# NVlabs/ODISE

Measured on NVIDIA H100. Metric: images/sec @1024x1024 panoptic inference (ODISE hot path), higher is better.
Workload: dtype f16q8

## Files before the change

odise_b200/csrc/gemm_tc.cu:

```cuda
#include "ptx.cuh"
#include "wgmma.cuh"
#include "odise_b200.h"
#include "launch_count.h"
#include <cudaTypedefs.h>
#include <mutex>
#include <map>
#include <cstring>
#include <vector>
#include <cstdlib>
#include <cstdio>

namespace ob {

struct GemmParams {
  int M, N, K, batch;
  int a_batched, b_batched;
  int conv, C, H, W, bw, bh, bb;
  int nseg;
  int cstride, cpad;
  int tiles_m, tiles_n, splits, kblocks;
  float alpha;
  const float* bias;
  const float* bias_m;
  const float* rowbias;
// ... 129 lines not shown
    float* d = p.D + (long long)z * p.d_bs + (long long)m * p.ldd + n;
    if (vec) {
      *reinterpret_cast<float4*>(d) = make_float4(acc[0], acc[1], acc[2], acc[3]);
    } else {
#pragma unroll
      for (int j = 0; j < 4; ++j) if (j < valid) d[j] = acc[j];
    }
  }
  if (p.Dh) {
    __nv_bfloat16* dh = p.Dh + (long long)z * p.h_bs + (long long)m * p.ldh + n;
    __nv_bfloat16* dl = p.Dl ? p.Dl + (long long)z * p.h_bs + (long long)m * p.ldh + n : nullptr;
    if (p.h16) {
      __align__(8) __nv_bfloat16 h[4];
      __align__(8) __nv_bfloat16 l[4];
#pragma unroll
      for (int t = 0; t < 4; ++t)
        split_f16(acc[t], *reinterpret_cast<uint16_t*>(&h[t]), *reinterpret_cast<uint16_t*>(&l[t]));
      if (vec) {
        *reinterpret_cast<uint2*>(dh) = *reinterpret_cast<const uint2*>(h);
        if (dl) *reinterpret_cast<uint2*>(dl) = *reinterpret_cast<const uint2*>(l);
      } else {
#pragma unroll
        for (int j = 0; j < 4; ++j) if (j < valid) { dh[j] = h[j]; if (dl) dl[j] = l[j]; }
      }
    } else if (vec) {
      store_planes<4>(dh, dl, acc);
    } else {
#pragma unroll
      for (int j = 0; j < 4; ++j) if (j < valid) store_planes<1>(dh + j, dl ? dl + j : nullptr, acc + j);
    }
  }
}

template <int BN, int NMMA>
struct GemmCfg {
  static constexpr int BM = 128, BK = 64;
  static constexpr int A_BYTES = BM * BK * 2;
  static constexpr int B_BYTES = BN * BK * 2;
  static constexpr int PLANES = (NMMA == 1) ? 1 : 2;
  static constexpr int STAGE_BYTES = PLANES * (A_BYTES + B_BYTES);
  static constexpr int THREADS = 384;
  static constexpr int EPI_BYTES = 8 * 32 * 16 * 4;
  static constexpr int STAGES_RAW = (232448 - EPI_BYTES - 256 - 1024) / STAGE_BYTES;
  static constexpr int STAGES = STAGES_RAW > 8 ? 8 : STAGES_RAW;
  static constexpr int SMEM_BYTES = STAGES * STAGE_BYTES + EPI_BYTES + 256 + 1024;
  static_assert(STAGES >= 2, "GEMM tile does not fit shared memory");
};

template <int BN, int NMMA, int EPI>
__global__ void __launch_bounds__(GemmCfg<BN, NMMA>::THREADS, 1)
gemm_tc_kernel(const __grid_constant__ CUtensorMap tmAh, const __grid_constant__ CUtensorMap tmAl,
               const __grid_constant__ CUtensorMap tmBh, const __grid_constant__ CUtensorMap tmBl, const GemmParams p) {
  using Cfg = GemmCfg<BN, NMMA>;
  extern __shared__ uint8_t smem_raw[];
  uint8_t* smem = reinterpret_cast<uint8_t*>((reinterpret_cast<uintptr_t>(smem_raw) + 1023) & ~uintptr_t(1023));
  float* epi_smem = reinterpret_cast<float*>(smem + Cfg::STAGES * Cfg::STAGE_BYTES);
  uint64_t* bars = reinterpret_cast<uint64_t*>(smem + Cfg::STAGES * Cfg::STAGE_BYTES + Cfg::EPI_BYTES);
  uint64_t* full = bars;
  uint64_t* empty = bars + Cfg::STAGES;

  const int warp = threadIdx.x >> 5;
  const int lane = threadIdx.x & 31;

  if (warp == 8 && lane == 0) {
    tma_prefetch_desc(&tmAh);
    tma_prefetch_desc(&tmBh);
    if (NMMA != 1) {
      tma_prefetch_desc(&tmAl);
      tma_prefetch_desc(&tmBl);
    }
    for (int s = 0; s < Cfg::STAGES; ++s) {
      mbar_init(&full[s], 1);
      mbar_init(&empty[s], 8);
    }
    fence_barrier_init();
  }
  __syncthreads();

  const int tiles_per_z = p.tiles_m * p.tiles_n * p.splits;
  const int total_tiles = tiles_per_z * p.batch;
  const int kb_per_split = (p.kblocks + p.splits - 1) / p.splits;

  if (warp >= 8) {
    setmaxnreg_dec<40>();
    if (warp == 8 && lane == 0) {
      int stage = 0;
      uint32_t phase = 0;
      const int cpk = p.conv ? (p.C / 64) : 1;
      for (int tile = blockIdx.x; tile < total_tiles; tile += gridDim.x) {
        const int z = tile / tiles_per_z;
        int r = tile - z * tiles_per_z;
        const int sp = r / (p.tiles_m * p.tiles_n);
        r -= sp * (p.tiles_m * p.tiles_n);
        const int mt = r / p.tiles_n, nt = r % p.tiles_n;
        const int m0 = mt * 128, n0 = nt * BN;
        const int kb0 = sp * kb_per_split;
        const int kb1 = min(p.kblocks, kb0 + kb_per_split);
        int b0 = 0, h0 = 0, w0 = 0;
        if (p.conv) {
          const int hw = p.H * p.W;
          b0 = m0 / hw;
          const int rem = m0 - b0 * hw;
          h0 = rem / p.W;
          w0 = rem - h0 * p.W;
        }
        for (int kb = kb0; kb < kb1; ++kb) {
          mbar_wait(&empty[stage], phase ^ 1);
          uint8_t* st = smem + stage * Cfg::STAGE_BYTES;
          mbar_arrive_expect_tx(&full[stage], Cfg::STAGE_BYTES);
          if (p.conv) {
            const int tap = kb / cpk, cc = kb - tap * cpk;
            const int kh = tap / 3, kw = tap - kh * 3;
            if (p.nseg == 1) {
              const int cx = w0 * p.cstride + kw - p.cpad, cy = h0 * p.cstride + kh - p.cpad;
              tma_load_4d(st, &tmAh, &full[stage], cc * 64, cx, cy, b0);
              if (NMMA != 1) tma_load_4d(st + Cfg::A_BYTES, &tmAl, &full[stage], cc * 64, cx, cy, b0);
            } else {
              const int hw = p.H * p.W;
              for (int sg = 0; sg < p.nseg; ++sg) {
                const int m = m0 + sg * p.bw;
                const int bi = m / hw, rem = m - bi * hw;
                const int hi_ = rem / p.W, wi = rem - hi_ * p.W;
                const int cx = wi * p.cstride + kw - p.cpad, cy = hi_ * p.cstride + kh - p.cpad;
                uint8_t* sa = st + sg * p.bw * 128;
                tma_load_4d(sa, &tmAh, &full[stage], cc * 64, cx, cy, bi);
                if (NMMA != 1) tma_load_4d(sa + Cfg::A_BYTES, &tmAl, &full[stage], cc * 64, cx, cy, bi);
              }
            }
          } else {
            const int za = p.a_batched ? z : 0;
            tma_load_3d(st, &tmAh, &full[stage], kb * 64, m0, za);
            if (NMMA != 1) tma_load_3d(st + Cfg::A_BYTES, &tmAl, &full[stage], kb * 64, m0, za);
          }
          const int zb = p.b_batched ? z : 0;
          uint8_t* sb = st + Cfg::PLANES * Cfg::A_BYTES;
          tma_load_3d(sb, &tmBh, &full[stage], kb * 64, n0, zb);
          if (NMMA != 1) tma_load_3d(sb + Cfg::B_BYTES, &tmBl, &full[stage], kb * 64, n0, zb);
          if (++stage == Cfg::STAGES) { stage = 0; phase ^= 1; }
        }
      }
    }
    return;
  }

  setmaxnreg_inc<232>();
  const int wg = warp >> 2, wi = warp & 3;
  int stage = 0;
  uint32_t phase = 0;
  float acc[BN / 2];
  float acc2[BN / 2];
  float* stg_wg = epi_smem + wg * (4 * 512);
  float* stg = stg_wg + wi * 512;
  const int cq = lane & 3, rsub = lane >> 2;
  for (int tile = blockIdx.x; tile < total_tiles; tile += gridDim.x) {
    const int z = tile / tiles_per_z;
    int r = tile - z * tiles_per_z;
    const int sp = r / (p.tiles_m * p.tiles_n);
    r -= sp * (p.tiles_m * p.tiles_n);
    const int mt = r / p.tiles_n, nt = r % p.tiles_n;
    const int n0 = nt * BN;
    const int kb0 = sp * kb_per_split;
    const int kb1 = min(p.kblocks, kb0 + kb_per_split);

    if (kb0 >= kb1) {
#pragma unroll
      for (int i = 0; i < BN / 2; ++i) acc[i] = 0.f;
      if constexpr (NMMA == 2) {
#pragma unroll
        for (int i = 0; i < BN / 2; ++i) acc2[i] = 0.f;
      }
    }
    int prev = -1;
    for (int kb = kb0; kb < kb1; ++kb) {
      mbar_wait(&full[stage], phase);
      const uint32_t sa = smem_u32(smem + stage * Cfg::STAGE_BYTES) + wg * (64 * 128);
      const uint32_t sb = smem_u32(smem + stage * Cfg::STAGE_BYTES + Cfg::PLANES * Cfg::A_BYTES);
      reg_fence(acc);
      if constexpr (NMMA == 2) reg_fence(acc2);
      wgmma_fence();
#pragma unroll
      for (int k = 0; k < 4; ++k) {
        const uint64_t a_hi = wgmma_desc_sw128(sa + k * 32);
        const uint64_t b_hi = wgmma_desc_sw128(sb + k * 32);
        const int accum = (kb > kb0 || k > 0) ? 1 : 0;
        if constexpr (NMMA == 2) wgmma_f16(acc, a_hi, b_hi, accum);
        else wgmma_bf16(acc, a_hi, b_hi, accum);
        if constexpr (NMMA == 3) {
          wgmma_bf16(acc, a_hi, wgmma_desc_sw128(sb + Cfg::B_BYTES + k * 32), 1);
          wgmma_bf16(acc, wgmma_desc_sw128(sa + Cfg::A_BYTES + k * 32), b_hi, 1);
        }
      }
      if constexpr (NMMA == 2) {
        const uint32_t a2 = sa + Cfg::A_BYTES, b2 = sb + Cfg::B_BYTES;
#pragma unroll
        for (int k = 0; k < 2; ++k) {
          wgmma_e5m2(acc2, wgmma_desc_sw128(a2 + k * 32), wgmma_desc_sw128(b2 + 64 + k * 32), (kb > kb0 || k > 0) ? 1 : 0);
          wgmma_e5m2(acc2, wgmma_desc_sw128(a2 + 64 + k * 32), wgmma_desc_sw128(b2 + k * 32), 1);
        }
      }
      wgmma_commit();
      wgmma_wait<1>();
      if (prev >= 0 && lane == 0) mbar_arrive(&empty[prev]);
      prev = stage;
      if (++stage == Cfg::STAGES) { stage = 0; phase ^= 1; }
    }
    wgmma_wait<0>();
    reg_fence(acc);
    if (prev >= 0 && lane == 0) mbar_arrive(&empty[prev]);
    if constexpr (NMMA == 2) {
      reg_fence(acc2);
#pragma unroll
      for (int i = 0; i < BN / 2; ++i) acc[i] += acc2[i];
    }

    const int m_base = mt * 128 + wg * 64 + (wi & 1) * 32;
    const bool interior = p.vec_ok && p.splits == 1 && (mt * 128 + 128 <= p.M) && (n0 + BN <= p.N);
    constexpr bool EXTRA = EPI == 1, GEGLU = EPI == 2;
    const bool has_bias = p.bias != nullptr, has_res = EXTRA && p.res != nullptr;
    const bool to_f32 = p.D != nullptr, to_hi = p.Dh != nullptr, to_lo = p.Dl != nullptr;
    const int act = p.act;
    const float alpha = p.alpha;
    const bool has_gn = !GEGLU && p.gnp != nullptr;
    const long long gn_seg = ((long long)z * p.M + m_base) >> 5;
#pragma unroll 1
    for (int ch = 0; ch < BN / 32; ++ch) {
      named_bar_sync(1 + wg, 128);
#pragma unroll
      for (int j = 0; j < BN / 8; ++j) {
        if ((j >> 2) != ch) continue;
#pragma unroll
        for (int h = 0; h < 2; ++h) {
          const int rw = wi * 16 + rsub + 8 * h, cc = 8 * (j & 3) + 2 * cq;
          const int rr = rw & 31, c16 = cc & 15;
          float* dst = stg_wg + ((rw >> 5) | ((cc >> 4) << 1)) * 512 + rr * 16 + (((c16 >> 2) ^ ((rr >> 1) & 3)) << 2) + (c16 & 3);
          *reinterpret_cast<float2*>(dst) = make_float2(acc[4 * j + 2 * h], acc[4 * j + 2 * h + 1]);
        }
      }
      named_bar_sync(1 + wg, 128);
      const int c0 = ch * 32 + (wi >> 1) * 16;
      if (interior) {
        GnAcc gacc;
        float4 b4 = make_float4(0.f, 0.f, 0.f, 0.f);
        if (has_bias) b4 = __ldg(reinterpret_cast<const float4*>(p.bias + n0 + c0 + cq * 4));
        float4 q[4];
#pragma unroll
        for (int it = 0; it < 4; ++it) {
          const int rr = it * 8 + rsub;
          q[it] = *reinterpret_cast<const float4*>(stg + rr * 16 + ((cq ^ ((rr >> 1) & 3)) << 2));
        }
        const int nn = n0 + c0 + cq * 4;
        float4 r4[4];
        if (has_res) {
#pragma unroll
          for (int it = 0; it < 4; ++it)
            r4[it] = *reinterpret_cast<const float4*>(p.res + (long long)z * p.res_bs + (long long)(m_base + it * 8 + rsub) * p.ldres + nn);
        }
#pragma unroll
        for (int it = 0; it < 4; ++it) {
          const long long m = m_base + it * 8 + rsub;
          float e[4] = {q[it].x, q[it].y, q[it].z, q[it].w};
          const float bb[4] = {b4.x, b4.y, b4.z, b4.w};
          const float bm = (EXTRA && p.bias_m) ? __ldg(p.bias_m + m) : 0.f;
#pragma unroll
          for (int j = 0; j < 4; ++j) e[j] = fmaf(e[j], alpha, EXTRA ? bb[j] + bm : bb[j]);
          if (EXTRA && p.rowbias) {
            const float4 rb = __ldg(reinterpret_cast<const float4*>(
                p.rowbias + (((long long)z * p.M + m) / p.rows_per_group) * p.rowbias_ld + nn));
            e[0] += rb.x; e[1] += rb.y; e[2] += rb.z; e[3] += rb.w;
          }
          if (GEGLU) {
            const bool odd = cq & 1;
            const float r0 = __shfl_xor_sync(0xffffffffu, odd ? e[0] : e[2], 1);
            const float r1 = __shfl_xor_sync(0xffffffffu, odd ? e[1] : e[3], 1);
            const float a0 = odd ? r0 : e[0], a1 = odd ? r1 : e[1];
            const float g0 = odd ? e[2] : r0, g1 = odd ? e[3] : r1;
            const float gv[2] = {a0 * gelu_erf_fast(g0), a1 * gelu_erf_fast(g1)};
            const long long og = (long long)z * p.h_bs + m * p.ldh + ((n0 + c0) >> 1) + (cq >> 1) * 4 + (odd ? 2 : 0);
            store_planes<2>(p.Dh + og, to_lo ? p.Dl + og : nullptr, gv);
            continue;
          }
          if (act != ODISE_ACT_NONE) {
#pragma unroll
            for (int j = 0; j < 4; ++j) e[j] = apply_act(e[j], act);
          }
          if (has_res) { e[0] += r4[it].x; e[1] += r4[it].y; e[2] += r4[it].z; e[3] += r4[it].w; }
          if (has_gn) gn_acc_rows(gacc, e, it == 0, lane);
          if (to_f32) *reinterpret_cast<float4*>(p.D + (long long)z * p.d_bs + m * p.ldd + nn) = make_float4(e[0], e[1], e[2], e[3]);
          const long long oh = (long long)z * p.h_bs + m * p.ldh + nn;
          if (to_hi && p.h16) {
            const __half2 h01 = __floats2half2_rn(e[0], e[1]), h23 = __floats2half2_rn(e[2], e[3]);
            uint2 hv;
            hv.x = *reinterpret_cast<const uint32_t*>(&h01);
            hv.y = *reinterpret_cast<const uint32_t*>(&h23);
            *reinterpret_cast<uint2*>(p.Dh + oh) = hv;
            if (to_lo) {
              const float2 f01 = __half22float2(h01), f23 = __half22float2(h23);
              const __half2 l01 = __floats2half2_rn(e[0] - f01.x, e[1] - f01.y);
              const __half2 l23 = __floats2half2_rn(e[2] - f23.x, e[3] - f23.y);
              uint2 lv;
              lv.x = *reinterpret_cast<const uint32_t*>(&l01);
              lv.y = *reinterpret_cast<const uint32_t*>(&l23);
              *reinterpret_cast<uint2*>(p.Dl + oh) = lv;
            }
          } else if (to_hi) {
            store_planes<4>(p.Dh + oh, to_lo ? p.Dl + oh : nullptr, e);
          }
        }
        if (has_gn) gn_acc_store(gacc, p, gn_seg, n0 + c0 + cq * 4, 4, lane);
      } else if (n0 + c0 < p.N) {
        const bool gn_here = p.gnp != nullptr && !p.geglu && p.splits == 1 && m_base < p.M;
        GnAcc gacc;
#pragma unroll 1
        for (int it = 0; it < 4; ++it) {
          const int rr = it * 8 + rsub;
          const float4 q4 = *reinterpret_cast<const float4*>(stg + rr * 16 + ((cq ^ ((rr >> 1) & 3)) << 2));
          const int m = m_base + rr, n = n0 + c0 + cq * 4;
          if (p.geglu) {
            float e[4] = {q4.x, q4.y, q4.z, q4.w};
#pragma unroll
            for (int j = 0; j < 4; ++j) e[j] = fmaf(e[j], p.alpha, p.bias ? __ldg(p.bias + n + j) : 0.f);
            float gt[4];
#pragma unroll
            for (int j = 0; j < 4; ++j) gt[j] = __shfl_xor_sync(0xffffffffu, e[j], 1);
            if ((cq & 1) == 0 && m < p.M) {
              float gv[4];
#pragma unroll
              for (int t = 0; t < 4; ++t) gv[t] = e[t] * gelu_erf_fast(gt[t]);
              const long long og = (long long)z * p.h_bs + (long long)m * p.ldh + ((n0 + c0) >> 1) + (cq >> 1) * 4;
              store_planes<4>(p.Dh + og, p.Dl ? p.Dl + og : nullptr, gv);
            }
            continue;
          }
          float fin[4] = {0.f, 0.f, 0.f, 0.f};
          if (m < p.M && n < p.N) {
            const int valid = min(4, p.N - n);
            if (p.splits > 1) {
              float* dst = p.partial + ((long long)(sp * p.batch + z) * p.M + m) * p.N + n;
              const float e[4] = {q4.x, q4.y, q4.z, q4.w};
#pragma unroll
              for (int j = 0; j < 4; ++j) if (j < valid) dst[j] = e[j];
            } else {
              epilogue_quad(p, z, m, n, valid, q4, fin);
            }
          }
          if (gn_here) gn_acc_rows(gacc, fin, it == 0, lane);
        }
        if (gn_here) {
          const int n = n0 + c0 + cq * 4;
          gn_acc_store(gacc, p, ((long long)z * p.M + m_base) >> 5, n, n < p.N ? min(4, p.N - n) : 0, lane);
        }
      }
    }
  }
}

__global__ void gemm_splitk_reduce_kernel(const GemmParams p) {
  const int quads = (p.N + 3) / 4;
  const long long total = (long long)p.batch * p.M * quads;
  for (long long i = blockIdx.x * (long long)blockDim.x + threadIdx.x; i < total;
       i += (long long)gridDim.x * blockDim.x) {
    const int qd = (int)(i % quads);
    const long long zm = i / quads;
    const int m = (int)(zm % p.M);
    const int z = (int)(zm / p.M);
    const int n = qd * 4;
    const int valid = min(4, p.N - n);
    float acc[4] = {0.f, 0.f, 0.f, 0.f};
    for (int sp = 0; sp < p.splits; ++sp) {
      const float* src = p.partial + ((long long)(sp * p.batch + z) * p.M + m) * p.N + n;
#pragma unroll
      for (int j = 0; j < 4; ++j) if (j < valid) acc[j] += src[j];
    }
    epilogue_quad(p, z, m, n, valid, make_float4(acc[0], acc[1], acc[2], acc[3]));
  }
}

static PFN_cuTensorMapEncodeTiled_v12000 get_encode() {
  static PFN_cuTensorMapEncodeTiled_v12000 fn = nullptr;
  static std::once_flag once;
  std::call_once(once, [] {
    void* f = nullptr;
    cudaDriverEntryPointQueryResult q;
    if (cudaGetDriverEntryPoint("cuTensorMapEncodeTiled", &f, cudaEnableDefault, &q) == cudaSuccess &&
        q == cudaDriverEntryPointSuccess)
      fn = reinterpret_cast<PFN_cuTensorMapEncodeTiled_v12000>(f);
  });
  return fn;
}

static int encode_map(CUtensorMap* tm, const void* base, int rank, const cuuint64_t* dims,
                      const cuuint64_t* strides_bytes, const cuuint32_t* box, int spatial_stride = 1) {
  auto enc = get_encode();
  if (!enc) return ODISE_ERR_DRIVER;
  cuuint32_t estr[5] = {1, (cuuint32_t)spatial_stride, (cuuint32_t)spatial_stride, 1, 1};
  CUresult r = enc(tm, CU_TENSOR_MAP_DATA_TYPE_BFLOAT16, rank, const_cast<void*>(base), dims, strides_bytes, box,
                   estr, CU_TENSOR_MAP_INTERLEAVE_NONE, CU_TENSOR_MAP_SWIZZLE_128B,
                   CU_TENSOR_MAP_L2_PROMOTION_L2_256B, CU_TENSOR_MAP_FLOAT_OOB_FILL_NONE);
  return r == CUDA_SUCCESS ? ODISE_OK : ODISE_ERR_TENSORMAP;
}

struct ProfRec { cudaEvent_t a, b; double flops; int M, N, K, batch, conv, bn, nmma, splits; };
static std::vector<ProfRec> g_prof;
static bool g_prof_on = false;

int num_sms() {
  static int n = 0;
  if (!n) {
    int dev = 0;
    cudaGetDevice(&dev);
    cudaDeviceGetAttribute(&n, cudaDevAttrMultiProcessorCount, dev);
    if (n <= 0) n = 132;
  }
  return n;
}

template <int BN, int NMMA, int EPI>
static int launch_cfg(const CUtensorMap& ah, const CUtensorMap& al, const CUtensorMap& bh, const CUtensorMap& bl,
                      const GemmParams& p, cudaStream_t stream) {
  using Cfg = GemmCfg<BN, NMMA>;
  static bool attr_set = false;
  if (!attr_set) {
    cudaError_t e = cudaFuncSetAttribute(gemm_tc_kernel<BN, NMMA, EPI>, cudaFuncAttributeMaxDynamicSharedMemorySize,
                                         Cfg::SMEM_BYTES);
    if (e != cudaSuccess) return (int)e;
    attr_set = true;
  }
  const int total = p.tiles_m * p.tiles_n * p.splits * p.batch;
  const int grid = total < num_sms() ? total : num_sms();
  gemm_tc_kernel<BN, NMMA, EPI><<<grid, Cfg::THREADS, Cfg::SMEM_BYTES, stream>>>(ah, al, bh, bl, p);
  return (int)cudaGetLastError();
}

static int pick_tile(int M, int N, int K, int batch, int forced, bool conv, int nmma) {
  const int cands[4] = {256, 160, 128, 64};
  const double eff[4] = {0.833, 0.933, 1.0, 1.333};
  const double epi_k = 480.0;
  const long long tm = (M + 127) / 128;
  double best = 1e30;
  int c = 128;
  for (int i = 0; i < 4; ++i) {
    const int bn = cands[i];
    if (forced && bn != forced) continue;
    if (nmma == 2 && bn > 128) continue;
    const long long tn = (N + bn - 1) / bn;
    const long long units = tm * tn * batch;
    const long long waves = (units + num_sms() - 1) / num_sms();
    double cost;
    if (conv) {
      cost = (double)waves * bn * eff[i] + 0.02 * bn;
    } else {
      const double mma = (double)bn * K * eff[i], epi = (double)bn * epi_k;
      cost = (double)waves * ((mma > epi ? mma : epi) + 20000.0);
    }
    if (cost < best) { best = cost; c = bn; }
  }
  return c;
}

}

using namespace ob;

// ... 91 lines not shown
    if (d->lda % 8 || d->a_batch_stride % 8) return ODISE_ERR_ALIGN;
    const long long bs = d->a_batch_stride ? d->a_batch_stride : (long long)d->M * d->lda;
    cuuint64_t dims[3] = {(cuuint64_t)d->K, (cuuint64_t)d->M, (cuuint64_t)(d->a_batch_stride ? d->batch : 1)};
    cuuint64_t str[2] = {(cuuint64_t)d->lda * 2, (cuuint64_t)bs * 2};
    cuuint32_t box[3] = {64, 128, 1};
    rc = encode_map(&ah, d->a_hi, 3, dims, str, box);
    if (rc) return rc;
    if (d->nmma == 2) {
      dims[0] = (cuuint64_t)((d->K + 63) / 64 * 64);
      if ((long long)dims[0] > d->lda) return ODISE_ERR_ALIGN;
    }
    rc = encode_map(&al, d->nmma != 1 ? d->a_lo : d->a_hi, 3, dims, str, box);
    if (rc) return rc;
  }
  p.tiles_m = (d->M + 127) / 128;
  if (d->ldb % 8 || d->b_batch_stride % 8) return ODISE_ERR_ALIGN;
  if (d->nmma == 2 && (long long)((d->K + 63) / 64 * 64) > d->ldb) return ODISE_ERR_ALIGN;
  if (d->geglu) {
    if (!d->out_hi || d->out_f32 || d->residual || d->rowbias || d->bias_m || d->split_k > 1 || d->N % 16 ||
        !p.vec_ok || d->act != ODISE_ACT_NONE)
      return ODISE_ERR_UNSUPPORTED;
  }
  p.kblocks = (d->K + 63) / 64;
  p.splits = d->split_k > 1 ? d->split_k : 1;
  if (p.splits > p.kblocks) p.splits = p.kblocks;
  if (p.splits > 1) {
    if (!d->workspace ||
        d->workspace_bytes < (long long)p.splits * d->batch * d->M * d->N * (long long)sizeof(float))
      return ODISE_ERR_WORKSPACE;
    p.partial = reinterpret_cast<float*>(d->workspace);
  }
  const int epi = d->geglu ? 2 : ((d->residual || d->rowbias || d->bias_m) ? 1 : 0);

  auto launch_with = [&](int bn) -> int {
    p.tiles_n = (d->N + bn - 1) / bn;
    const long long bs = d->b_batch_stride ? d->b_batch_stride : (long long)d->N * d->ldb;
    cuuint64_t dims[3] = {(cuuint64_t)d->K, (cuuint64_t)d->N, (cuuint64_t)(d->b_batch_stride ? d->batch : 1)};
    cuuint64_t str[2] = {(cuuint64_t)d->ldb * 2, (cuuint64_t)bs * 2};
    cuuint32_t box[3] = {64, (cuuint32_t)bn, 1};
    int r = encode_map(&bh, d->b_hi, 3, dims, str, box);
    if (r) return r;
    if (d->nmma == 2) dims[0] = (cuuint64_t)((d->K + 63) / 64 * 64);
    r = encode_map(&bl, d->nmma != 1 ? d->b_lo : d->b_hi, 3, dims, str, box);
    if (r) return r;
#define ODISE_LAUNCH(BN_, NM_)                                                   \
  r = epi == 2   ? launch_cfg<BN_, NM_, 2>(ah, al, bh, bl, p, stream)            \
      : epi == 1 ? launch_cfg<BN_, NM_, 1>(ah, al, bh, bl, p, stream)            \
                 : launch_cfg<BN_, NM_, 0>(ah, al, bh, bl, p, stream)
    if (d->nmma == 3) {
      switch (bn) {
        case 64: ODISE_LAUNCH(64, 3); break;
        case 128: ODISE_LAUNCH(128, 3); break;
        case 160: ODISE_LAUNCH(160, 3); break;
        default: ODISE_LAUNCH(256, 3); break;
      }
    } else if (d->nmma == 2) {
      if (bn == 64) ODISE_LAUNCH(64, 2);
      else ODISE_LAUNCH(128, 2);
    } else {
      switch (bn) {
        case 64: ODISE_LAUNCH(64, 1); break;
        case 128: ODISE_LAUNCH(128, 1); break;
        case 160: ODISE_LAUNCH(160, 1); break;
        default: ODISE_LAUNCH(256, 1); break;
      }
    }
#undef ODISE_LAUNCH
    if (r) return r;
    if (p.splits > 1) {
      const long long total = (long long)p.batch * p.M * ((p.N + 3) / 4);
      int blocks = (int)((total + 127) / 128);
      if (blocks > num_sms() * 8) blocks = num_sms() * 8;
      gemm_splitk_reduce_kernel<<<blocks, 128, 0, stream>>>(p);
      r = (int)cudaGetLastError();
    }
    return r;
  };

  int BN;
  {
    static const bool tune = !(getenv("ODISE_GEMM_AUTOTUNE") && atoi(getenv("ODISE_GEMM_AUTOTUNE")) == 0);
    const int fbn = (d->force_bn == 64 || d->force_bn == 128 || d->force_bn == 160 || d->force_bn == 256) ? d->force_bn : 0;
    BN = pick_tile(d->M, d->N, d->K, d->batch, fbn, d->conv3x3 != 0, d->nmma);
    struct Key {
      int v[13];
      bool operator<(const Key& o) const { return memcmp(v, o.v, sizeof(v)) < 0; }
    };
    static std::map<Key, int> cache;
    static std::mutex mu;
    const Key key{{d->M, d->N, d->K, d->batch, d->conv3x3 ? 1 + d->conv_mode : 0, d->conv_W, d->nmma, epi, p.splits,
                  (d->out_f32 ? 1 : 0) | (d->out_hi ? 2 : 0) | (d->out_planes_fp16 << 2), p.gnp ? 1 : 0, d->act, p.vec_ok}};
    cudaStreamCaptureStatus cap = cudaStreamCaptureStatusNone;
    cudaStreamIsCapturing(stream, &cap);
    std::lock_guard<std::mutex> lk(mu);
    auto it = cache.find(key);
    if (it != cache.end()) {
      BN = it->second;
    } else if (tune && !fbn && !g_prof_on && cap == cudaStreamCaptureStatusNone &&
               !(d->residual && (const void*)d->residual == (const void*)d->out_f32)) {
      const int cands[4] = {256, 160, 128, 64};
      cudaEvent_t e0, e1;
      cudaEventCreate(&e0);
      cudaEventCreate(&e1);
      float best = 1e30f;
      int bc = BN;
      for (int i = 0; i < 4; ++i) {
        const int c = cands[i];
        if (c == 64 && d->N > 96 && (long long)p.tiles_m * ((d->N + 127) / 128) * d->batch >= 2 * num_sms()) continue;
        if (c > 128 && (d->N <= 64 || d->nmma == 2)) continue;
        if (launch_with(c)) { (void)cudaGetLastError(); continue; }
        cudaEventRecord(e0, stream);
        int r2 = launch_with(c);
        if (!r2) r2 = launch_with(c);
        cudaEventRecord(e1, stream);
        if (r2 || cudaEventSynchronize(e1) != cudaSuccess) { (void)cudaGetLastError(); continue; }
        float ms = 0.f;
        cudaEventElapsedTime(&ms, e0, e1);
        if (ms < best) { best = ms; bc = c; }
      }
      cudaEventDestroy(e0);
      cudaEventDestroy(e1);
      cache[key] = bc;
      BN = bc;
      if (getenv("ODISE_VERBOSE"))
        fprintf(stderr, "odise_b200: gemm %d x %d x %d (batch %d, conv %d, nmma %d, epi %d): BN %d, %.1f us\n", d->M, d->N,
                d->K, d->batch, d->conv3x3, d->nmma, epi, BN, best * 500.f);
    }
  }

  ProfRec rec{};
  if (g_prof_on) {
    cudaEventCreate(&rec.a);
    cudaEventCreate(&rec.b);
    rec.flops = 2.0 * d->M * d->N * (double)d->K * d->batch;
    rec.M = d->M; rec.N = d->N; rec.K = d->K; rec.batch = d->batch; rec.conv = d->conv3x3; rec.bn = BN;
    rec.nmma = d->nmma; rec.splits = p.splits;
    cudaEventRecord(rec.a, stream);
  }
  rc = launch_with(BN);
  if (rc) return rc;
  count_launch(p.splits > 1 ? 2 : 1);
  if (g_prof_on) {
    cudaEventRecord(rec.b, stream);
    g_prof.push_back(rec);
  }
  return rc;
}

extern "C" int odise_gemm_tile_policy(int M, int N, int K, int batch, int conv3x3, int nmma, int* bn, int* pair) {
  if (M <= 0 || N <= 0 || K <= 0 || batch <= 0 || !bn || !pair || nmma < 1 || nmma > 3) return ODISE_ERR_ARG;
  *bn = pick_tile(M, N, K, batch, 0, conv3x3 != 0, nmma);
  *pair = 0;
  return ODISE_OK;
}

extern "C" int odise_profile_begin(void) {
  for (auto& r : g_prof) { cudaEventDestroy(r.a); cudaEventDestroy(r.b); }
  g_prof.clear();
  g_prof_on = true;
  return ODISE_OK;
}

extern "C" int odise_profile_end(long long* launches, double* total_ms, double* total_flops) {
  g_prof_on = false;
  cudaError_t e = cudaDeviceSynchronize();
  if (e != cudaSuccess) return (int)e;
  double ms = 0, fl = 0;
  FILE* fcsv = nullptr;
  if (const char* path = getenv("ODISE_PROFILE_CSV")) fcsv = fopen(path, "a");
  if (fcsv) fprintf(fcsv, "M,N,K,batch,conv,bn,nmma,splits,ms,tflops\n");
  for (auto& r : g_prof) {
    float t = 0;
// ... 16 lines not shown
```

Before: 12.41.

## Add warp-specialized epilogue variant that hands accumulators to dedicated epilogue warps

Adds a HAND variant of the TMA/WGMMA GEMM. Consumer warpgroups dump accumulator chunks into shared-memory slots guarded by mbarriers. Three otherwise idle producer-group warps then run the bias/activation/residual/GN epilogue, with residual loads prefetched before waiting, so the epilogue overlaps the next tile's MMAs. The autotuner now times both variants per BN, and the extra staging slots can reduce pipeline stages, and register rebalancing via setmaxnreg is skipped in this mode.

```diff
diff --git a/odise_b200/csrc/gemm_tc.cu b/odise_b200/csrc/gemm_tc.cu
--- a/odise_b200/csrc/gemm_tc.cu
+++ b/odise_b200/csrc/gemm_tc.cu
@@ -185,7 +185,7 @@
   }
 }
 
-template <int BN, int NMMA>
+template <int BN, int NMMA, bool HAND>
 struct GemmCfg {
   static constexpr int BM = 128, BK = 64;
   static constexpr int A_BYTES = BM * BK * 2;
@@ -193,24 +193,164 @@
   static constexpr int PLANES = (NMMA == 1) ? 1 : 2;
   static constexpr int STAGE_BYTES = PLANES * (A_BYTES + B_BYTES);
   static constexpr int THREADS = 384;
+  static constexpr int EPI_WARPS = 3;
+  static constexpr int SLOT_BYTES = BM * 32 * 4;
+  static constexpr int TILE_SLOTS = BN / 32;
   static constexpr int EPI_BYTES = 8 * 32 * 16 * 4;
-  static constexpr int STAGES_RAW = (232448 - EPI_BYTES - 256 - 1024) / STAGE_BYTES;
-  static constexpr int STAGES = STAGES_RAW > 8 ? 8 : STAGES_RAW;
-  static constexpr int SMEM_BYTES = STAGES * STAGE_BYTES + EPI_BYTES + 256 + 1024;
-  static_assert(STAGES >= 2, "GEMM tile does not fit shared memory");
+  static constexpr int AVAIL = 232448 - 256 - 1024;
+  static constexpr int cap8(int s) { return s > 8 ? 8 : s; }
+  static constexpr int STAGES_MAX = cap8((AVAIL - (HAND ? 2 * SLOT_BYTES : EPI_BYTES)) / STAGE_BYTES);
+  static constexpr int STAGES_TILE = (AVAIL - TILE_SLOTS * SLOT_BYTES) / STAGE_BYTES;
+  static constexpr int STAGES_FLOOR = STAGES_MAX < 4 ? STAGES_MAX : 4;
+  static constexpr int STAGES_FIT = STAGES_TILE < STAGES_MAX ? STAGES_TILE : STAGES_MAX;
+  static constexpr int STAGES = !HAND ? STAGES_MAX : (STAGES_FIT > STAGES_FLOOR ? STAGES_FIT : STAGES_FLOOR);
+  static constexpr int SLOTS_RAW = (AVAIL - STAGES * STAGE_BYTES) / SLOT_BYTES;
+  static constexpr int SLOTS = !HAND ? 0 : (SLOTS_RAW < TILE_SLOTS ? SLOTS_RAW : TILE_SLOTS);
+  static constexpr int STAGING_BYTES = HAND ? SLOTS * SLOT_BYTES : EPI_BYTES;
+  static constexpr int SMEM_BYTES = STAGES * STAGE_BYTES + STAGING_BYTES + 256 + 1024;
+  static_assert(STAGES >= 2 && (!HAND || SLOTS >= 2), "GEMM tile does not fit shared memory");
+  static_assert(2 * (STAGES + SLOTS) * 8 <= 256, "barrier area");
 };
 
-template <int BN, int NMMA, int EPI>
-__global__ void __launch_bounds__(GemmCfg<BN, NMMA>::THREADS, 1)
+template <int EPI, bool PRE>
+__device__ __forceinline__ void epilogue_block(const GemmParams& p, const float* stg, int z, int sp, int m_base, int n0,
+                                               int c0, bool interior, const float4 (&r4_in)[4], int lane) {
+  const int cq = lane & 3, rsub = lane >> 2;
+  constexpr bool EXTRA = EPI == 1, GEGLU = EPI == 2;
+  const bool has_bias = p.bias != nullptr, has_res = EXTRA && p.res != nullptr;
+  const bool to_f32 = p.D != nullptr, to_hi = p.Dh != nullptr, to_lo = p.Dl != nullptr;
+  const int act = p.act;
+  const float alpha = p.alpha;
+  const bool has_gn = !GEGLU && p.gnp != nullptr;
+  const long long gn_seg = ((long long)z * p.M + m_base) >> 5;
+  if (interior) {
+    GnAcc gacc;
+    float4 b4 = make_float4(0.f, 0.f, 0.f, 0.f);
+    if (has_bias) b4 = __ldg(reinterpret_cast<const float4*>(p.bias + n0 + c0 + cq * 4));
+    float4 q[4];
+#pragma unroll
+    for (int it = 0; it < 4; ++it) {
+      const int rr = it * 8 + rsub;
+      q[it] = *reinterpret_cast<const float4*>(stg + rr * 16 + ((cq ^ ((rr >> 1) & 3)) << 2));
+    }
+    const int nn = n0 + c0 + cq * 4;
+    float4 r4[4];
+#pragma unroll
+    for (int it = 0; it < 4; ++it) {
+      if (PRE) r4[it] = r4_in[it];
+      else if (has_res)
+        r4[it] = *reinterpret_cast<const float4*>(p.res + (long long)z * p.res_bs + (long long)(m_base + it * 8 + rsub) * p.ldres + nn);
+    }
+#pragma unroll
+    for (int it = 0; it < 4; ++it) {
+      const long long m = m_base + it * 8 + rsub;
+      float e[4] = {q[it].x, q[it].y, q[it].z, q[it].w};
+      const float bb[4] = {b4.x, b4.y, b4.z, b4.w};
+      const float bm = (EXTRA && p.bias_m) ? __ldg(p.bias_m + m) : 0.f;
+#pragma unroll
+      for (int j = 0; j < 4; ++j) e[j] = fmaf(e[j], alpha, EXTRA ? bb[j] + bm : bb[j]);
+      if (EXTRA && p.rowbias) {
+        const float4 rb = __ldg(reinterpret_cast<const float4*>(
+            p.rowbias + (((long long)z * p.M + m) / p.rows_per_group) * p.rowbias_ld + nn));
+        e[0] += rb.x; e[1] += rb.y; e[2] += rb.z; e[3] += rb.w;
+      }
+      if (GEGLU) {
+        const bool odd = cq & 1;
+        const float r0 = __shfl_xor_sync(0xffffffffu, odd ? e[0] : e[2], 1);
+        const float r1 = __shfl_xor_sync(0xffffffffu, odd ? e[1] : e[3], 1);
+        const float a0 = odd ? r0 : e[0], a1 = odd ? r1 : e[1];
+        const float g0 = odd ? e[2] : r0, g1 = odd ? e[3] : r1;
+        const float gv[2] = {a0 * gelu_erf_fast(g0), a1 * gelu_erf_fast(g1)};
+        const long long og = (long long)z * p.h_bs + m * p.ldh + ((n0 + c0) >> 1) + (cq >> 1) * 4 + (odd ? 2 : 0);
+        store_planes<2>(p.Dh + og, to_lo ? p.Dl + og : nullptr, gv);
+        continue;
+      }
+      if (act != ODISE_ACT_NONE) {
+#pragma unroll
+        for (int j = 0; j < 4; ++j) e[j] = apply_act(e[j], act);
+      }
+      if (has_res) { e[0] += r4[it].x; e[1] += r4[it].y; e[2] += r4[it].z; e[3] += r4[it].w; }
+      if (has_gn) gn_acc_rows(gacc, e, it == 0, lane);
+      if (to_f32) *reinterpret_cast<float4*>(p.D + (long long)z * p.d_bs + m * p.ldd + nn) = make_float4(e[0], e[1], e[2], e[3]);
+      const long long oh = (long long)z * p.h_bs + m * p.ldh + nn;
+      if (to_hi && p.h16) {
+        const __half2 h01 = __floats2half2_rn(e[0], e[1]), h23 = __floats2half2_rn(e[2], e[3]);
+        uint2 hv;
+        hv.x = *reinterpret_cast<const uint32_t*>(&h01);
+        hv.y = *reinterpret_cast<const uint32_t*>(&h23);
+        *reinterpret_cast<uint2*>(p.Dh + oh) = hv;
+        if (to_lo) {
+          const float2 f01 = __half22float2(h01), f23 = __half22float2(h23);
+          const __half2 l01 = __floats2half2_rn(e[0] - f01.x, e[1] - f01.y);
+          const __half2 l23 = __floats2half2_rn(e[2] - f23.x, e[3] - f23.y);
+          uint2 lv;
+          lv.x = *reinterpret_cast<const uint32_t*>(&l01);
+          lv.y = *reinterpret_cast<const uint32_t*>(&l23);
+          *reinterpret_cast<uint2*>(p.Dl + oh) = lv;
+        }
+      } else if (to_hi) {
+        store_planes<4>(p.Dh + oh, to_lo ? p.Dl + oh : nullptr, e);
+      }
+    }
+    if (has_gn) gn_acc_store(gacc, p, gn_seg, n0 + c0 + cq * 4, 4, lane);
+  } else if (n0 + c0 < p.N) {
+    const bool gn_here = p.gnp != nullptr && !p.geglu && p.splits == 1 && m_base < p.M;
+    GnAcc gacc;
+#pragma unroll 1
+    for (int it = 0; it < 4; ++it) {
+      const int rr = it * 8 + rsub;
+      const float4 q4 = *reinterpret_cast<const float4*>(stg + rr * 16 + ((cq ^ ((rr >> 1) & 3)) << 2));
+      const int m = m_base + rr, n = n0 + c0 + cq * 4;
+      if (p.geglu) {
+        float e[4] = {q4.x, q4.y, q4.z, q4.w};
+#pragma unroll
+        for (int j = 0; j < 4; ++j) e[j] = fmaf(e[j], p.alpha, p.bias ? __ldg(p.bias + n + j) : 0.f);
+        float gt[4];
+#pragma unroll
+        for (int j = 0; j < 4; ++j) gt[j] = __shfl_xor_sync(0xffffffffu, e[j], 1);
+        if ((cq & 1) == 0 && m < p.M) {
+          float gv[4];
+#pragma unroll
+          for (int t = 0; t < 4; ++t) gv[t] = e[t] * gelu_erf_fast(gt[t]);
+          const long long og = (long long)z * p.h_bs + (long long)m * p.ldh + ((n0 + c0) >> 1) + (cq >> 1) * 4;
+          store_planes<4>(p.Dh + og, p.Dl ? p.Dl + og : nullptr, gv);
+        }
+        continue;
+      }
+      float fin[4] = {0.f, 0.f, 0.f, 0.f};
+      if (m < p.M && n < p.N) {
+        const int valid = min(4, p.N - n);
+        if (p.splits > 1) {
+          float* dst = p.partial + ((long long)(sp * p.batch + z) * p.M + m) * p.N + n;
+          const float e[4] = {q4.x, q4.y, q4.z, q4.w};
+#pragma unroll
+          for (int j = 0; j < 4; ++j) if (j < valid) dst[j] = e[j];
+        } else {
+          epilogue_quad(p, z, m, n, valid, q4, fin);
+        }
+      }
+      if (gn_here) gn_acc_rows(gacc, fin, it == 0, lane);
+    }
+    if (gn_here) {
+      const int n = n0 + c0 + cq * 4;
+      gn_acc_store(gacc, p, gn_seg, n, n < p.N ? min(4, p.N - n) : 0, lane);
+    }
+  }
+}
+
+template <int BN, int NMMA, int EPI, bool HAND>
+__global__ void __launch_bounds__(GemmCfg<BN, NMMA, HAND>::THREADS, 1)
 gemm_tc_kernel(const __grid_constant__ CUtensorMap tmAh, const __grid_constant__ CUtensorMap tmAl,
                const __grid_constant__ CUtensorMap tmBh, const __grid_constant__ CUtensorMap tmBl, const GemmParams p) {
-  using Cfg = GemmCfg<BN, NMMA>;
+  using Cfg = GemmCfg<BN, NMMA, HAND>;
   extern __shared__ uint8_t smem_raw[];
   uint8_t* smem = reinterpret_cast<uint8_t*>((reinterpret_cast<uintptr_t>(smem_raw) + 1023) & ~uintptr_t(1023));
-  float* epi_smem = reinterpret_cast<float*>(smem + Cfg::STAGES * Cfg::STAGE_BYTES);
-  uint64_t* bars = reinterpret_cast<uint64_t*>(smem + Cfg::STAGES * Cfg::STAGE_BYTES + Cfg::EPI_BYTES);
+  float* acc_smem = reinterpret_cast<float*>(smem + Cfg::STAGES * Cfg::STAGE_BYTES);
+  uint64_t* bars = reinterpret_cast<uint64_t*>(smem + Cfg::STAGES * Cfg::STAGE_BYTES + Cfg::STAGING_BYTES);
   uint64_t* full = bars;
-  uint64_t* empty = bars + Cfg::STAGES;
+  uint64_t* empty = full + Cfg::STAGES;
+  uint64_t* acc_full = empty + Cfg::STAGES;
+  uint64_t* acc_empty = acc_full + Cfg::SLOTS;
 
   const int warp = threadIdx.x >> 5;
   const int lane = threadIdx.x & 31;
@@ -226,6 +366,10 @@
       mbar_init(&full[s], 1);
       mbar_init(&empty[s], 8);
     }
+    for (int s = 0; s < Cfg::SLOTS; ++s) {
+      mbar_init(&acc_full[s], 256);
+      mbar_init(&acc_empty[s], 32 * Cfg::EPI_WARPS);
+    }
     fence_barrier_init();
   }
   __syncthreads();
@@ -233,10 +377,12 @@
   const int tiles_per_z = p.tiles_m * p.tiles_n * p.splits;
   const int total_tiles = tiles_per_z * p.batch;
   const int kb_per_split = (p.kblocks + p.splits - 1) / p.splits;
+  const int cq = lane & 3, rsub = lane >> 2;
 
   if (warp >= 8) {
-    setmaxnreg_dec<40>();
-    if (warp == 8 && lane == 0) {
+  if constexpr (!HAND) setmaxnreg_dec<40>();
+  if (warp == 8) {
+    if (lane == 0) {
       int stage = 0;
       uint32_t phase = 0;
       const int cpk = p.conv ? (p.C / 64) : 1;
@@ -296,22 +442,66 @@
     return;
   }
 
-  setmaxnreg_inc<232>();
+  {
+    if constexpr (!HAND) return;
+    constexpr int EW = Cfg::EPI_WARPS, PER = (8 + EW - 1) / EW;
+    constexpr bool EXTRA = EPI == 1;
+    const int ew = warp - 9;
+    int slot = 0, rot = 0;
+    uint32_t slot_phase = 0;
+    for (int tile = blockIdx.x; tile < total_tiles; tile += gridDim.x) {
+      const int z = tile / tiles_per_z;
+      int r = tile - z * tiles_per_z;
+      const int sp = r / (p.tiles_m * p.tiles_n);
+      r -= sp * (p.tiles_m * p.tiles_n);
+      const int mt = r / p.tiles_n, nt = r % p.tiles_n;
+      const int n0 = nt * BN;
+      const bool interior = p.vec_ok && p.splits == 1 && (mt * 128 + 128 <= p.M) && (n0 + BN <= p.N);
+      const bool pre_res = interior && EXTRA && p.res != nullptr;
+#pragma unroll 1
+      for (int ch = 0; ch < BN / 32; ++ch) {
+        const int b0 = (ew - rot + EW) % EW;
+        rot = (rot + 8) % EW;
+        float4 r4[PER][4];
+#pragma unroll
+        for (int i = 0; i < PER; ++i) {
+          const int b = b0 + i * EW;
+          if (pre_res && b < 8) {
+            const long long m = mt * 128 + (b & 3) * 32 + rsub;
+            const int nn = n0 + ch * 32 + (b >> 2) * 16 + cq * 4;
+#pragma unroll
+            for (int it = 0; it < 4; ++it)
+              r4[i][it] = *reinterpret_cast<const float4*>(p.res + (long long)z * p.res_bs + (m + it * 8) * p.ldres + nn);
+          }
+        }
+        mbar_wait(&acc_full[slot], slot_phase);
+        const float* sl = acc_smem + slot * (Cfg::SLOT_BYTES / 4);
+#pragma unroll
+        for (int i = 0; i < PER; ++i) {
+          const int b = b0 + i * EW;
+          if (b < 8)
+            epilogue_block<EPI, true>(p, sl + b * 512, z, sp, mt * 128 + (b & 3) * 32, n0, ch * 32 + (b >> 2) * 16, interior,
+                                r4[i], lane);
+        }
+        mbar_arrive(&acc_empty[slot]);
+        if (++slot == Cfg::SLOTS) { slot = 0; slot_phase ^= 1; }
+      }
+    }
+    return;
+  }
+  }
+
+  if constexpr (!HAND) setmaxnreg_inc<232>();
   const int wg = warp >> 2, wi = warp & 3;
   int stage = 0;
   uint32_t phase = 0;
+  int slot = 0;
+  uint32_t slot_phase = 0;
   float acc[BN / 2];
   float acc2[BN / 2];
-  float* stg_wg = epi_smem + wg * (4 * 512);
-  float* stg = stg_wg + wi * 512;
-  const int cq = lane & 3, rsub = lane >> 2;
   for (int tile = blockIdx.x; tile < total_tiles; tile += gridDim.x) {
     const int z = tile / tiles_per_z;
-    int r = tile - z * tiles_per_z;
-    const int sp = r / (p.tiles_m * p.tiles_n);
-    r -= sp * (p.tiles_m * p.tiles_n);
-    const int mt = r / p.tiles_n, nt = r % p.tiles_n;
-    const int n0 = nt * BN;
+    const int sp = (tile - z * tiles_per_z) / (p.tiles_m * p.tiles_n);
     const int kb0 = sp * kb_per_split;
     const int kb1 = min(p.kblocks, kb0 + kb_per_split);
 
@@ -366,142 +556,49 @@
       for (int i = 0; i < BN / 2; ++i) acc[i] += acc2[i];
     }
 
-    const int m_base = mt * 128 + wg * 64 + (wi & 1) * 32;
-    const bool interior = p.vec_ok && p.splits == 1 && (mt * 128 + 128 <= p.M) && (n0 + BN <= p.N);
-    constexpr bool EXTRA = EPI == 1, GEGLU = EPI == 2;
-    const bool has_bias = p.bias != nullptr, has_res = EXTRA && p.res != nullptr;
-    const bool to_f32 = p.D != nullptr, to_hi = p.Dh != nullptr, to_lo = p.Dl != nullptr;
-    const int act = p.act;
-    const float alpha = p.alpha;
-    const bool has_gn = !GEGLU && p.gnp != nullptr;
-    const long long gn_seg = ((long long)z * p.M + m_base) >> 5;
+    if constexpr (HAND) {
+      const int rr = (wi & 1) * 16 + rsub, x = (cq >> 1) ^ ((rr >> 1) & 3);
+      const int base = (wg * 2 + (wi >> 1)) * 512 + rr * 16 + 2 * (cq & 1);
+      const int off[2] = {base + (x << 2), base + ((x ^ 2) << 2)};
+#pragma unroll
+      for (int ch = 0; ch < BN / 32; ++ch) {
+        mbar_wait(&acc_empty[slot], slot_phase ^ 1);
+        float* sl = acc_smem + slot * (Cfg::SLOT_BYTES / 4);
+#pragma unroll
+        for (int jj = 0; jj < 4; ++jj) {
+          const int j = ch * 4 + jj;
+#pragma unroll
+          for (int h = 0; h < 2; ++h)
+            *reinterpret_cast<float2*>(sl + off[jj & 1] + (jj >> 1) * 2048 + h * 128) =
+                make_float2(acc[4 * j + 2 * h], acc[4 * j + 2 * h + 1]);
+        }
+        mbar_arrive(&acc_full[slot]);
+        if (++slot == Cfg::SLOTS) { slot = 0; slot_phase ^= 1; }
+      }
+    } else {
+      float* stg_wg = acc_smem + wg * (4 * 512);
+      int r = tile - z * tiles_per_z - sp * (p.tiles_m * p.tiles_n);
+      const int mt = r / p.tiles_n, n0 = (r % p.tiles_n) * BN;
+      const int m_base = mt * 128 + wg * 64 + (wi & 1) * 32;
+      const bool interior = p.vec_ok && p.splits == 1 && (mt * 128 + 128 <= p.M) && (n0 + BN <= p.N);
 #pragma unroll 1
-    for (int ch = 0; ch < BN / 32; ++ch) {
-      named_bar_sync(1 + wg, 128);
-#pragma unroll
-      for (int j = 0; j < BN / 8; ++j) {
-        if ((j >> 2) != ch) continue;
-#pragma unroll
-        for (int h = 0; h < 2; ++h) {
-          const int rw = wi * 16 + rsub + 8 * h, cc = 8 * (j & 3) + 2 * cq;
-          const int rr = rw & 31, c16 = cc & 15;
-          float* dst = stg_wg + ((rw >> 5) | ((cc >> 4) << 1)) * 512 + rr * 16 + (((c16 >> 2) ^ ((rr >> 1) & 3)) << 2) + (c16 & 3);
-          *reinterpret_cast<float2*>(dst) = make_float2(acc[4 * j + 2 * h], acc[4 * j + 2 * h + 1]);
-        }
-      }
-      named_bar_sync(1 + wg, 128);
-      const int c0 = ch * 32 + (wi >> 1) * 16;
-      if (interior) {
-        GnAcc gacc;
-        float4 b4 = make_float4(0.f, 0.f, 0.f, 0.f);
-        if (has_bias) b4 = __ldg(reinterpret_cast<const float4*>(p.bias + n0 + c0 + cq * 4));
-        float4 q[4];
-#pragma unroll
-        for (int it = 0; it < 4; ++it) {
-          const int rr = it * 8 + rsub;
-          q[it] = *reinterpret_cast<const float4*>(stg + rr * 16 + ((cq ^ ((rr >> 1) & 3)) << 2));
-        }
-        const int nn = n0 + c0 + cq * 4;
-        float4 r4[4];
-        if (has_res) {
-#pragma unroll
-          for (int it = 0; it < 4; ++it)
-            r4[it] = *reinterpret_cast<const float4*>(p.res + (long long)z * p.res_bs + (long long)(m_base + it * 8 + rsub) * p.ldres + nn);
-        }
-#pragma unroll
-        for (int it = 0; it < 4; ++it) {
-          const long long m = m_base + it * 8 + rsub;
-          float e[4] = {q[it].x, q[it].y, q[it].z, q[it].w};
-          const float bb[4] = {b4.x, b4.y, b4.z, b4.w};
-          const float bm = (EXTRA && p.bias_m) ? __ldg(p.bias_m + m) : 0.f;
-#pragma unroll
-          for (int j = 0; j < 4; ++j) e[j] = fmaf(e[j], alpha, EXTRA ? bb[j] + bm : bb[j]);
-          if (EXTRA && p.rowbias) {
-            const float4 rb = __ldg(reinterpret_cast<const float4*>(
-                p.rowbias + (((long long)z * p.M + m) / p.rows_per_group) * p.rowbias_ld + nn));
-            e[0] += rb.x; e[1] += rb.y; e[2] += rb.z; e[3] += rb.w;
-          }
-          if (GEGLU) {
-            const bool odd = cq & 1;
-            const float r0 = __shfl_xor_sync(0xffffffffu, odd ? e[0] : e[2], 1);
-            const float r1 = __shfl_xor_sync(0xffffffffu, odd ? e[1] : e[3], 1);
-            const float a0 = odd ? r0 : e[0], a1 = odd ? r1 : e[1];
-            const float g0 = odd ? e[2] : r0, g1 = odd ? e[3] : r1;
-            const float gv[2] = {a0 * gelu_erf_fast(g0), a1 * gelu_erf_fast(g1)};
-            const long long og = (long long)z * p.h_bs + m * p.ldh + ((n0 + c0) >> 1) + (cq >> 1) * 4 + (odd ? 2 : 0);
-            store_planes<2>(p.Dh + og, to_lo ? p.Dl + og : nullptr, gv);
-            continue;
-          }
-          if (act != ODISE_ACT_NONE) {
-#pragma unroll
-            for (int j = 0; j < 4; ++j) e[j] = apply_act(e[j], act);
-          }
-          if (has_res) { e[0] += r4[it].x; e[1] += r4[it].y; e[2] += r4[it].z; e[3] += r4[it].w; }
-          if (has_gn) gn_acc_rows(gacc, e, it == 0, lane);
-          if (to_f32) *reinterpret_cast<float4*>(p.D + (long long)z * p.d_bs + m * p.ldd + nn) = make_float4(e[0], e[1], e[2], e[3]);
-          const long long oh = (long long)z * p.h_bs + m * p.ldh + nn;
-          if (to_hi && p.h16) {
-            const __half2 h01 = __floats2half2_rn(e[0], e[1]), h23 = __floats2half2_rn(e[2], e[3]);
-            uint2 hv;
-            hv.x = *reinterpret_cast<const uint32_t*>(&h01);
-            hv.y = *reinterpret_cast<const uint32_t*>(&h23);
-            *reinterpret_cast<uint2*>(p.Dh + oh) = hv;
-            if (to_lo) {
-              const float2 f01 = __half22float2(h01), f23 = __half22float2(h23);
-              const __half2 l01 = __floats2half2_rn(e[0] - f01.x, e[1] - f01.y);
-              const __half2 l23 = __floats2half2_rn(e[2] - f23.x, e[3] - f23.y);
-              uint2 lv;
-              lv.x = *reinterpret_cast<const uint32_t*>(&l01);
-              lv.y = *reinterpret_cast<const uint32_t*>(&l23);
-              *reinterpret_cast<uint2*>(p.Dl + oh) = lv;
-            }
-          } else if (to_hi) {
-            store_planes<4>(p.Dh + oh, to_lo ? p.Dl + oh : nullptr, e);
+      for (int ch = 0; ch < BN / 32; ++ch) {
+        named_bar_sync(1 + wg, 128);
+#pragma unroll
+        for (int j = 0; j < BN / 8; ++j) {
+          if ((j >> 2) != ch) continue;
+#pragma unroll
+          for (int h = 0; h < 2; ++h) {
+            const int rw = wi * 16 + rsub + 8 * h, cc = 8 * (j & 3) + 2 * cq;
+            const int rr = rw & 31, c16 = cc & 15;
+            float* dst = stg_wg + ((rw >> 5) | ((cc >> 4) << 1)) * 512 + rr * 16 + (((c16 >> 2) ^ ((rr >> 1) & 3)) << 2) + (c16 & 3);
+            *reinterpret_cast<float2*>(dst) = make_float2(acc[4 * j + 2 * h], acc[4 * j + 2 * h + 1]);
           }
         }
-        if (has_gn) gn_acc_store(gacc, p, gn_seg, n0 + c0 + cq * 4, 4, lane);
-      } else if (n0 + c0 < p.N) {
-        const bool gn_here = p.gnp != nullptr && !p.geglu && p.splits == 1 && m_base < p.M;
-        GnAcc gacc;
-#pragma unroll 1
-        for (int it = 0; it < 4; ++it) {
-          const int rr = it * 8 + rsub;
-          const float4 q4 = *reinterpret_cast<const float4*>(stg + rr * 16 + ((cq ^ ((rr >> 1) & 3)) << 2));
-          const int m = m_base + rr, n = n0 + c0 + cq * 4;
-          if (p.geglu) {
-            float e[4] = {q4.x, q4.y, q4.z, q4.w};
-#pragma unroll
-            for (int j = 0; j < 4; ++j) e[j] = fmaf(e[j], p.alpha, p.bias ? __ldg(p.bias + n + j) : 0.f);
-            float gt[4];
-#pragma unroll
-            for (int j = 0; j < 4; ++j) gt[j] = __shfl_xor_sync(0xffffffffu, e[j], 1);
-            if ((cq & 1) == 0 && m < p.M) {
-              float gv[4];
-#pragma unroll
-              for (int t = 0; t < 4; ++t) gv[t] = e[t] * gelu_erf_fast(gt[t]);
-              const long long og = (long long)z * p.h_bs + (long long)m * p.ldh + ((n0 + c0) >> 1) + (cq >> 1) * 4;
-              store_planes<4>(p.Dh + og, p.Dl ? p.Dl + og : nullptr, gv);
-            }
-            continue;
-          }
-          float fin[4] = {0.f, 0.f, 0.f, 0.f};
-          if (m < p.M && n < p.N) {
-            const int valid = min(4, p.N - n);
-            if (p.splits > 1) {
-              float* dst = p.partial + ((long long)(sp * p.batch + z) * p.M + m) * p.N + n;
-              const float e[4] = {q4.x, q4.y, q4.z, q4.w};
-#pragma unroll
-              for (int j = 0; j < 4; ++j) if (j < valid) dst[j] = e[j];
-            } else {
-              epilogue_quad(p, z, m, n, valid, q4, fin);
-            }
-          }
-          if (gn_here) gn_acc_rows(gacc, fin, it == 0, lane);
-        }
-        if (gn_here) {
-          const int n = n0 + c0 + cq * 4;
-          gn_acc_store(gacc, p, ((long long)z * p.M + m_base) >> 5, n, n < p.N ? min(4, p.N - n) : 0, lane);
-        }
+        named_bar_sync(1 + wg, 128);
+        const int c0 = ch * 32 + (wi >> 1) * 16;
+        const float4 none[4] = {};
+        epilogue_block<EPI, false>(p, stg_wg + wi * 512, z, sp, m_base, n0, c0, interior, none, lane);
       }
     }
   }
@@ -567,20 +664,20 @@
   return n;
 }
 
-template <int BN, int NMMA, int EPI>
+template <int BN, int NMMA, int EPI, bool HAND>
 static int launch_cfg(const CUtensorMap& ah, const CUtensorMap& al, const CUtensorMap& bh, const CUtensorMap& bl,
                       const GemmParams& p, cudaStream_t stream) {
-  using Cfg = GemmCfg<BN, NMMA>;
+  using Cfg = GemmCfg<BN, NMMA, HAND>;
   static bool attr_set = false;
   if (!attr_set) {
-    cudaError_t e = cudaFuncSetAttribute(gemm_tc_kernel<BN, NMMA, EPI>, cudaFuncAttributeMaxDynamicSharedMemorySize,
+    cudaError_t e = cudaFuncSetAttribute(gemm_tc_kernel<BN, NMMA, EPI, HAND>, cudaFuncAttributeMaxDynamicSharedMemorySize,
                                          Cfg::SMEM_BYTES);
     if (e != cudaSuccess) return (int)e;
     attr_set = true;
   }
   const int total = p.tiles_m * p.tiles_n * p.splits * p.batch;
   const int grid = total < num_sms() ? total : num_sms();
-  gemm_tc_kernel<BN, NMMA, EPI><<<grid, Cfg::THREADS, Cfg::SMEM_BYTES, stream>>>(ah, al, bh, bl, p);
+  gemm_tc_kernel<BN, NMMA, EPI, HAND><<<grid, Cfg::THREADS, Cfg::SMEM_BYTES, stream>>>(ah, al, bh, bl, p);
   return (int)cudaGetLastError();
 }
 
@@ -738,7 +835,7 @@
   }
   const int epi = d->geglu ? 2 : ((d->residual || d->rowbias || d->bias_m) ? 1 : 0);
 
-  auto launch_with = [&](int bn) -> int {
+  auto launch_with = [&](int bn, bool hand) -> int {
     p.tiles_n = (d->N + bn - 1) / bn;
     const long long bs = d->b_batch_stride ? d->b_batch_stride : (long long)d->N * d->ldb;
     cuuint64_t dims[3] = {(cuuint64_t)d->K, (cuuint64_t)d->N, (cuuint64_t)(d->b_batch_stride ? d->batch : 1)};
@@ -749,10 +846,14 @@
     if (d->nmma == 2) dims[0] = (cuuint64_t)((d->K + 63) / 64 * 64);
     r = encode_map(&bl, d->nmma != 1 ? d->b_lo : d->b_hi, 3, dims, str, box);
     if (r) return r;
+#define ODISE_LAUNCH_H(BN_, NM_, H_)                                             \
+  r = epi == 2   ? launch_cfg<BN_, NM_, 2, H_>(ah, al, bh, bl, p, stream)        \
+      : epi == 1 ? launch_cfg<BN_, NM_, 1, H_>(ah, al, bh, bl, p, stream)        \
+                 : launch_cfg<BN_, NM_, 0, H_>(ah, al, bh, bl, p, stream)
 #define ODISE_LAUNCH(BN_, NM_)                                                   \
-  r = epi == 2   ? launch_cfg<BN_, NM_, 2>(ah, al, bh, bl, p, stream)            \
-      : epi == 1 ? launch_cfg<BN_, NM_, 1>(ah, al, bh, bl, p, stream)            \
-                 : launch_cfg<BN_, NM_, 0>(ah, al, bh, bl, p, stream)
+  do {                                                                           \
+    if (hand) { ODISE_LAUNCH_H(BN_, NM_, true); } else { ODISE_LAUNCH_H(BN_, NM_, false); } \
+  } while (0)
     if (d->nmma == 3) {
       switch (bn) {
         case 64: ODISE_LAUNCH(64, 3); break;
@@ -772,6 +873,7 @@
       }
     }
 #undef ODISE_LAUNCH
+#undef ODISE_LAUNCH_H
     if (r) return r;
     if (p.splits > 1) {
       const long long total = (long long)p.batch * p.M * ((p.N + 3) / 4);
@@ -784,6 +886,7 @@
   };
 
   int BN;
+  bool HAND = false;
   {
     static const bool tune = !(getenv("ODISE_GEMM_AUTOTUNE") && atoi(getenv("ODISE_GEMM_AUTOTUNE")) == 0);
     const int fbn = (d->force_bn == 64 || d->force_bn == 128 || d->force_bn == 160 || d->force_bn == 256) ? d->force_bn : 0;
@@ -801,7 +904,8 @@
     std::lock_guard<std::mutex> lk(mu);
     auto it = cache.find(key);
     if (it != cache.end()) {
-      BN = it->second;
+      BN = it->second >> 1;
+      HAND = it->second & 1;
     } else if (tune && !fbn && !g_prof_on && cap == cudaStreamCaptureStatusNone &&
                !(d->residual && (const void*)d->residual == (const void*)d->out_f32)) {
       const int cands[4] = {256, 160, 128, 64};
@@ -809,28 +913,30 @@
       cudaEventCreate(&e0);
       cudaEventCreate(&e1);
       float best = 1e30f;
-      int bc = BN;
-      for (int i = 0; i < 4; ++i) {
-        const int c = cands[i];
+      int bc = 2 * BN;
+      for (int i = 0; i < 8; ++i) {
+        const int c = cands[i >> 1];
+        const bool h = i & 1;
         if (c == 64 && d->N > 96 && (long long)p.tiles_m * ((d->N + 127) / 128) * d->batch >= 2 * num_sms()) continue;
         if (c > 128 && (d->N <= 64 || d->nmma == 2)) continue;
-        if (launch_with(c)) { (void)cudaGetLastError(); continue; }
+        if (launch_with(c, h)) { (void)cudaGetLastError(); continue; }
         cudaEventRecord(e0, stream);
-        int r2 = launch_with(c);
-        if (!r2) r2 = launch_with(c);
+        int r2 = launch_with(c, h);
+        if (!r2) r2 = launch_with(c, h);
         cudaEventRecord(e1, stream);
         if (r2 || cudaEventSynchronize(e1) != cudaSuccess) { (void)cudaGetLastError(); continue; }
         float ms = 0.f;
         cudaEventElapsedTime(&ms, e0, e1);
-        if (ms < best) { best = ms; bc = c; }
+        if (ms < best) { best = ms; bc = 2 * c + h; }
       }
       cudaEventDestroy(e0);
       cudaEventDestroy(e1);
       cache[key] = bc;
-      BN = bc;
+      BN = bc >> 1;
+      HAND = bc & 1;
       if (getenv("ODISE_VERBOSE"))
-        fprintf(stderr, "odise_b200: gemm %d x %d x %d (batch %d, conv %d, nmma %d, epi %d): BN %d, %.1f us\n", d->M, d->N,
-                d->K, d->batch, d->conv3x3, d->nmma, epi, BN, best * 500.f);
+        fprintf(stderr, "odise_b200: gemm %d x %d x %d (batch %d, conv %d, nmma %d, epi %d): BN %d%s, %.1f us\n", d->M,
+                d->N, d->K, d->batch, d->conv3x3, d->nmma, epi, BN, HAND ? " (epilogue warps)" : "", best * 500.f);
     }
   }
 
@@ -843,7 +949,7 @@
     rec.nmma = d->nmma; rec.splits = p.splits;
     cudaEventRecord(rec.a, stream);
   }
-  rc = launch_with(BN);
+  rc = launch_with(BN, HAND);
   if (rc) return rc;
   count_launch(p.splits > 1 ? 2 : 1);
   if (g_prof_on) {
```

Measured after the change: 12.46, median of 6. No clear change (+0.4%).
